# arkCyber/whisper-rust

Measured on AMD Instinct MI355X. Metric: real-time factor (audio-sec/wall-sec), greedy, 30 s synthetic chunks, higher is better.
Workload: dtype f16 operands / f32 accumulate; 1 GPU; ggml-small-shaped synthetic F16 model, greedy best_of=1 temperature_inc=0, 1 x 30 s 16 kHz f32 chunk per GPU, PCM resident in HBM; flash_attn=False, parallelism=chunk-dp1

## Files before the change

### whisper-rust_amd/csrc/wa_device.h

```cpp
#pragma once
#include "wa_kernels.h"

#include <hip/hip_runtime.h>
#include <stdint.h>

typedef _Float16 h16;
typedef _Float16 half8 __attribute__((ext_vector_type(8)));
typedef _Float16 half2v __attribute__((ext_vector_type(2)));
typedef float    f32x4 __attribute__((ext_vector_type(4)));

#define WAVE 64

__device__ __forceinline__ float h2f(wa_f16 v) { union { wa_f16 u; h16 h; } c; c.u = v; return (float) c.h; }
__device__ __forceinline__ wa_f16 f2h(float v) { asm("" : "+v"(v)); union { wa_f16 u; h16 h; } c; c.h = (h16) v; return c.u; }

__device__ __forceinline__ void wa_barrier_lds() { asm volatile("s_waitcnt lgkmcnt(0)\n\ts_barrier" ::: "memory"); }

__device__ __forceinline__ float wave_sum(float v) {
#pragma unroll
    for (int o = 32; o > 0; o >>= 1) v += __shfl_xor(v, o, WAVE);
    return v;
}
template <int CTRL, int ROW_MASK = 0xf>
__device__ __forceinline__ float dpp_f32(float v) {
// ... 3 lines not shown
__device__ __forceinline__ double dpp_f64(double v) {
    const long long b = __builtin_bit_cast(long long, v);
    const int lo = __builtin_amdgcn_update_dpp(0, (int) (b & 0xffffffffll), CTRL, ROW_MASK, 0xf, true);
    const int hi = __builtin_amdgcn_update_dpp(0, (int) (b >> 32), CTRL, ROW_MASK, 0xf, true);
    return __builtin_bit_cast(double, ((long long) hi << 32) | (unsigned int) lo);
}
__device__ __forceinline__ double wave_sum_d(double v) {
    v += dpp_f64<0x111>(v);
    v += dpp_f64<0x112>(v);
    v += dpp_f64<0x114>(v);
    v += dpp_f64<0x118>(v);
    v += dpp_f64<0x142, 0xa>(v);
    v += dpp_f64<0x143, 0xc>(v);
    const long long b = __builtin_bit_cast(long long, v);
    const int lo = __builtin_amdgcn_readlane((int) (b & 0xffffffffll), 63), hi = __builtin_amdgcn_readlane((int) (b >> 32), 63);
    return __builtin_bit_cast(double, ((long long) hi << 32) | (unsigned int) lo);
}
__device__ __forceinline__ float wave_max(float v) {
#pragma unroll
    for (int o = 32; o > 0; o >>= 1) v = fmaxf(v, __shfl_xor(v, o, WAVE));
    return v;
}

__device__ __forceinline__ float wa_expf(float x) {
    const float r = 0x1.8p23f;
    const float z = fmaf(x, 0x1.715476p+0f, r);
    const float n = z - r;
    const float b = fmaf(-n, 0x1.7f7d1cp-20f, fmaf(-n, 0x1.62e4p-1f, x));
    const uint32_t e = __float_as_uint(z) << 23;
    const float k = __uint_as_float(e + __float_as_uint(1.0f));
    const float an = fabsf(n);
    const float u = b * b;
    const float j = fmaf(fmaf(fmaf(0x1.0e4020p-7f, b, 0x1.573e2ep-5f), u, fmaf(0x1.555e66p-3f, b, 0x1.fffdb6p-2f)), u,
                         0x1.ffffecp-1f * b);
    if (!(an > 126.0f)) return fmaf(j, k, k);
    const uint32_t g = (n <= 0.0f) ? 0x82000000u : 0u;
    const float s1 = __uint_as_float(g + 0x7f000000u);
    const float s2 = __uint_as_float(e - g);
    if (an > 192.0f) return s1 * s1;
    return fmaf(s2, j, s2) * s1;
}

__device__ __forceinline__ float wa_gelu_nb(float x, const wa_f16 * __restrict__ table) {
    const float t = h2f(table[f2h(x)]);
    return x <= -10.0f ? 0.0f : (x >= 10.0f ? x : t);
}
__device__ __forceinline__ float wa_gelu(float x, const wa_f16 * __restrict__ table) {
    if (x <= -10.0f) return 0.0f;
    if (x >=  10.0f) return x;
    return h2f(table[f2h(x)]);
}

__device__ __forceinline__ void wa_q8_store(float y, int row, int blk, int el, int nb, int8_t * __restrict__ qs, float * __restrict__ qd,
                                            float * __restrict__ qsum = nullptr) {
    float a = fabsf(y);
    a = fmaxf(a, dpp_f32<0x128>(a));
    a = fmaxf(a, dpp_f32<0x124>(a));
    a = fmaxf(a, dpp_f32<0x122>(a));
    a = fmaxf(a, dpp_f32<0x121>(a));
    a = fmaxf(a, __shfl_xor(a, 16, 32));
    const float d = a / 127.f;
    const float id = a != 0.0f ? 127.f / a : 0.0f;
    const int q = (int) rintf(y * id);
    qs[(((size_t) row * 8 + (el >> 2)) * nb + blk) * 4 + (el & 3)] = (int8_t) q;
    if (el == 0) qd[(size_t) row * nb + blk] = h2f(f2h(d));
    if (qsum) {
        int t = q;
        t += __builtin_amdgcn_update_dpp(0, t, 0x128, 0xf, 0xf, true);
        t += __builtin_amdgcn_update_dpp(0, t, 0x124, 0xf, 0xf, true);
        t += __builtin_amdgcn_update_dpp(0, t, 0x122, 0xf, 0xf, true);
        t += __builtin_amdgcn_update_dpp(0, t, 0x121, 0xf, 0xf, true);
        t += __shfl_xor(t, 16, 32);
        if (el == 0) qsum[(size_t) row * nb + blk] = h2f(f2h(d * (float) t));
    }
}

struct wa_epi_pre { float bias = 0.f, scale = 1.f, resid = 0.f; };

template <int EPI>
__device__ __forceinline__ wa_epi_pre epi_preload(const wa_epi & e, int m, int n) {
    wa_epi_pre p;
    if (e.bias) p.bias = e.bias[n];
    if ((EPI == WA_EPI_F16 || EPI == WA_EPI_CROSS_KV || EPI == WA_EPI_DEC_QKV) && e.scale) p.scale = e.scale[n];
    if (EPI == WA_EPI_RESID || EPI == WA_EPI_CONV2) p.resid = e.resid[(size_t) m * e.ldr + n];
    return p;
}

template <int EPI>
__device__ __forceinline__ void epi_apply(const wa_epi & e, int m, int n, float acc, const wa_epi_pre & p) {
    float v = acc;
    if (e.bias) v = v + p.bias;
    if (EPI == WA_EPI_F16) {
        if (e.scale) v = v * p.scale;
        ((wa_f16 *) e.out)[(size_t) m * e.ldo + n] = f2h(v);
    } else if (EPI == WA_EPI_ENC_QKV) {
        if (n < e.split0) ((wa_f16 *) e.out)[(size_t) m * e.ldo + n] = f2h(v);
        else              ((wa_f16 *) e.out2)[(size_t) (n - e.split0) * e.ldo2 + m] = f2h(v);
    } else if (EPI == WA_EPI_GELU_F16) {
        ((wa_f16 *) e.out)[(size_t) m * e.ldo + n] = f2h(wa_gelu(v, e.gelu));
    } else if (EPI == WA_EPI_GELU_F32) {
        ((float *) e.out)[(size_t) m * e.ldo + n] = wa_gelu(v, e.gelu);
    } else if (EPI == WA_EPI_RESID) {
        ((float *) e.out)[(size_t) m * e.ldo + n] = v + p.resid;
    } else if (EPI == WA_EPI_CONV2) {
        const float g = wa_gelu(v, e.gelu);
        if (e.dbg) e.dbg[(size_t) m * e.ldo + n] = g;
        ((float *) e.out)[(size_t) m * e.ldo + n] = p.resid + g;
    } else if (EPI == WA_EPI_F32) {
        ((float *) e.out)[(size_t) m * e.ldo + n] = v;
    } else if (EPI == WA_EPI_CROSS_KV) {
        if (e.scale) v = v * p.scale;
        const int d = e.aux1, two_d = 2 * d;
        const int il = n / two_d, r = n - il * two_d;
        const int kv = r >= d, rr = kv ? r - d : r;
        const int n_head = d >> 6, hd = rr >> 6, c = rr & 63;
        wa_f16 * dst = (wa_f16 *) (kv ? e.out2 : e.out);
        dst[(((size_t) il * n_head + hd) * e.aux0 + m) * 64 + c] = f2h(v);
    } else if (EPI == WA_EPI_DEC_QKV) {
        if (e.scale) v = v * p.scale;
        const int row_off = e.dyn ? e.dyn[1] : e.row_off;
        if (n < e.split0)      ((wa_f16 *) e.out)[(size_t) m * e.ldo + n] = f2h(v);
        else if (e.rowp) {
            const wa_rowptr r = e.rowp[m];
            if (n < e.split1) (r.kv_k + e.rowp_off)[(size_t) r.kv_head * e.ldo2 + (n - e.split0)] = f2h(v);
            else              (r.kv_v + e.rowp_off)[(size_t) r.kv_head * e.ldo3 + (n - e.split1)] = f2h(v);
        }
        else if (n < e.split1) ((wa_f16 *) e.out2)[(size_t) (row_off + m) * e.ldo2 + (n - e.split0)] = f2h(v);
        else                   ((wa_f16 *) e.out3)[(size_t) (row_off + m) * e.ldo3 + (n - e.split1)] = f2h(v);
    }
}

template <int EPI>
__device__ __forceinline__ void epi_store(const wa_epi & e, int m, int n, float acc) {
    epi_apply<EPI>(e, m, n, acc, epi_preload<EPI>(e, m, n));
}

__device__ __forceinline__ float wa_tree32(const float (&s)[32]) {
    float a[8];
#pragma unroll
    for (int l = 0; l < 8; ++l) a[l] = (s[l] + s[16 + l]) + (s[8 + l] + s[24 + l]);
    const float t0 = a[0] + a[4], t1 = a[1] + a[5], t2 = a[2] + a[6], t3 = a[3] + a[7];
    return (t0 + t1) + (t2 + t3);
}

static __device__ const unsigned long long WA_EXP2F_T[32] = {
    0x3ff0000000000000ULL, 0x3fefd9b0d3158574ULL, 0x3fefb5586cf9890fULL, 0x3fef9301d0125b51ULL, 0x3fef72b83c7d517bULL,
    0x3fef54873168b9aaULL, 0x3fef387a6e756238ULL, 0x3fef1e9df51fdee1ULL, 0x3fef06fe0a31b715ULL, 0x3feef1a7373aa9cbULL,
    0x3feedea64c123422ULL, 0x3feece086061892dULL, 0x3feebfdad5362a27ULL, 0x3feeb42b569d4f82ULL, 0x3feeab07dd485429ULL,
    0x3feea47eb03a5585ULL, 0x3feea09e667f3bcdULL, 0x3fee9f75e8ec5f74ULL, 0x3feea11473eb0187ULL, 0x3feea589994cce13ULL,
    0x3feeace5422aa0dbULL, 0x3feeb737b0cdc5e5ULL, 0x3feec49182a3f090ULL, 0x3feed503b23e255dULL, 0x3feee89f995ad3adULL,
    0x3feeff76f2fb5e47ULL, 0x3fef199bdd85529cULL, 0x3fef3720dcef9069ULL, 0x3fef5818dcfba487ULL, 0x3fef7c97337b9b5fULL,
    0x3fefa4afa2a490daULL, 0x3fefd0765b6e4540ULL,
};
__device__ __forceinline__ float wa_expf_libm(float x) {
    if (!(x >= -0x1.9fe368p6f)) return 0.0f;
    const double InvLn2N = 0x1.71547652b82fep+0 * 32;
    const double C0 = 0x1.c6af84b912394p-5 / 32 / 32 / 32, C1 = 0x1.ebfce50fac4f3p-3 / 32 / 32, C2 = 0x1.62e42ff0c52d6p-1 / 32;
    const double SHIFT = 0x1.8p+52;
    double z = InvLn2N * (double) x;
    double kd = z + SHIFT;
    const unsigned long long ki = (unsigned long long) __double_as_longlong(kd);
    kd = kd - SHIFT;
    const double r = z - kd;
    const unsigned long long t = WA_EXP2F_T[ki & 31] + (ki << 47);
    const double s = __longlong_as_double((long long) t);
    z = fma(C0, r, C1);
    const double r2 = r * r;
    double y = fma(C2, r, 1.0);
    y = fma(z, r2, y);
    y = y * s;
    return (float) y;
}

__device__ __forceinline__ bool wa_sum_bounds(double S, double A, int n, float & lo, float & hi, double rn) {
    const double delta = (2.0 * (double) n * 0x1p-53 * A + fabs(S) * 0x1p-48) * rn * 1.000001;
    const double q = S * rn;
    lo = (float) (q - delta); hi = (float) (q + delta);
    return lo == hi;
}
__device__ __forceinline__ bool wa_sum_certain(double S, double A, int n, float & out, double rn) { float hi; return wa_sum_bounds(S, A, n, out, hi, rn); }
__device__ __forceinline__ bool wa_sum_certain(double S, double A, int n, float & out) { return wa_sum_certain(S, A, n, out, 1.0 / (double) n); }
__device__ __forceinline__ bool wa_mean_indifferent(float x, float lo, float hi) { return (x - lo) == (x - hi); }

__device__ __forceinline__ void wa_softmax_bounds(double tot, int ng, float & ilo, float & ihi) {
    const double delta = (double) (ng + 8 + 16) * 0x1p-53 * tot * 1.000001;
    ilo = (float) (1.0 / (tot + delta)); ihi = (float) (1.0 / (tot - delta));
}

__device__ __forceinline__ double wa_seq_sum_lds(const float * row, int d, bool squares, float mean) {
    double t = 0.0;
    int i = 0;
    for (; i + 4 <= d; i += 4) {
        const float4 v = *(const float4 *) (row + i);
        if (!squares) { t += (double) v.x; t += (double) v.y; t += (double) v.z; t += (double) v.w; }
        else {
            const float a = v.x - mean, b = v.y - mean, c = v.z - mean, e = v.w - mean;
            t += (double) (a * a); t += (double) (b * b); t += (double) (c * c); t += (double) (e * e);
        }
    }
    for (; i < d; ++i) { const float a = row[i] - mean; t += squares ? (double) (a * a) : (double) row[i]; }
    return t;
}
```

### whisper-rust_amd/csrc/wa_mega.hip

```cpp
#include "wa_one_launch_dev.h"
#include "wa_mega.h"

typedef const __attribute__((address_space(4))) wa_mega_args * mg_kargs;

#define MG_THREADS 512
#define MG_NW (MG_THREADS / 64)
#define MG_NP3 4

__device__ __forceinline__ int mq_fresh(int) {
    unsigned z = 0; asm volatile("" : "+v"(z));
    return (int) __builtin_amdgcn_mbcnt_hi(~0u, __builtin_amdgcn_mbcnt_lo(~0u, z));
}
__device__ __forceinline__ void mq_put(float y, bool act, unsigned * q32, float * dsc, int lane) {
    float dq;
    const unsigned w = mq_quant32(y, dq);
    if (act && (lane & 3) == 0) *q32 = w;
    if (act && (lane & 31) == 0) *dsc = dq;
}

__device__ __forceinline__ gu64 * mg_edge(mg_kargs A, int layer, int e) {
    return (gu64 *) A->granules + ((size_t) layer * WA_MEGA_EDGES + e) * A->edge_stride;
}

__device__ __forceinline__ int8_t * mq_xq(wa_f16 * xin) { return (int8_t *) xin; }
// ... 750 lines not shown
                    v = v + t.bias;
                    float gl = v;
                    if (v <= -10.0f) gl = 0.0f; else if (v < 10.0f) gl = h2f(gelu_l[t.valid ? f2h(v) : 0]);
                    if constexpr (Q) { if (t.valid && (lane & 7) == 0) gr_store(eh + t.row, seq, __float_as_uint(gl)); }
                    else mg_pub_h2(eh, seq, t.valid, t.row, (unsigned) f2h(gl), lane);
                }
                mg_trace(A, wg == 0 && wave == 1 && lane == 0, (l * 8 + 4) * 8 + 3, mg_now());
                if ((wave == 3 || wave == 4) && wave - 1 < g_ff) big_next(wave);
                else if (wave >= 6 && l + 1 >= L) mg_prefetch_logits<NS, Q>(A, pf, have_pf, lane, wave);
            }
        } else
        if (wave == 1 || wave == 2 || (BIG && (wave == 3 || wave == 4))) {
            bool assisted = false;
            gu64 * eh = mg_edge(A, l, E_HF);
            for (int grp = wave - 1; grp < g_ff; grp += BIG ? 4 : 2) {
                if (grp >= 2) { t = mg_mk8<Q, NS>(pf, Y.fc1_w, Y.fc1_d, Y.fc1_b, nullptr, d4, d, row_ff, r_ff, grp, lane); assisted = true; }
                MG_CHAOS_AT(7u);
                float v = mg_do8<Q, NS>(pf, t, d >> 5, xinB, lane);
                v = v + t.bias;
                float gl = v;
                if (v <= -10.0f) gl = 0.0f; else if (v < 10.0f) gl = h2f(gelu_l[t.valid ? f2h(v) : 0]);
                if constexpr (Q) { if (t.valid && (lane & 7) == 0) gr_store(eh + t.row, seq, __float_as_uint(gl)); }
                else mg_pub_h2(eh, seq, t.valid, t.row, (unsigned) f2h(gl), lane);
            }
            mg_trace(A, wg == 0 && wave == 1 && lane == 0, (l * 8 + 4) * 8 + 3, mg_now());
            if (A->dbg && l == MG_WGTRACE_LAYER) mg_trace(A, wave == 1 && lane == 0, 4096 + wg * 8 + 6, mg_now());
            if (CQ) {
                if (l + 1 >= L) mg_prefetch_logits<NS, Q>(A, pf, have_pf, lane, wave);
            } else if (assisted) {
                if (l + 1 >= L) mg_prefetch_logits<NS, Q>(A, pf, have_pf, lane, wave);
                else t = wave == 3 ? mg_mk8<Q, NS>(pf, Ly[l + 1].out_w, Ly[l + 1].out_d, Ly[l + 1].out_b, nullptr, d, d, row_d, r_d, 0, lane)
                                   : mg_mk8<Q, NS>(pf, Ly[l + 1].cq_w, Ly[l + 1].cq_d, Ly[l + 1].cq_b, nullptr, d, d, row_d, r_d, 0, lane);
            }
        }
        MG_FRESH();
        {
            const int ng = QB ? 9 * (d4 >> 5) : Q ? d4 : 2 * d;
            const int qs = mg_slot(wave, QB || BIG ? MG_EX_HFQ : MG_EX_HF), sg = mg_seg(ng), i0 = qs * sg, i1 = min(ng, i0 + sg);
            if constexpr (QB) { if (qs >= 0) mg_gather_qb<3>(c, mg_edge(A, l, E_HF), i0, i1, lane, xin, d4 >> 5, 600u + l, A, wg == 0 && wave == 0 ? (l * 8 + 5) * 8 : -1); }
            else if constexpr (Q) { if (qs >= 0) mg_gather_q8<(NP3 == MG_NP3 ? 14 : 8)>(c, mg_edge(A, l, E_HF), i0, i1, lane, xin, d4 >> 5, 600u + l, A, wg == 0 && wave == 0 ? (l * 8 + 5) * 8 : -1); }
            else if (qs >= 0) mg_gather_h2<7>(c, mg_edge(A, l, E_HF), i0, i1, lane, (unsigned *) xin, 600u + l, A, wg == 0 && wave == 0 ? (l * 8 + 5) * 8 : -1);
        }
        wa_barrier_lds();
        MG_FRESH();
        mg_trace(A, wg == 0 && wave == 5 && lane == 0, (l * 8 + 5) * 8 + 4, mg_now());
        if (!CQ && (wave == 1 || wave == 2)) {
            if (l + 1 < L) t = mg_mk8<Q, NS>(pf, Ly[l + 1].qkv_w, Ly[l + 1].qkv_d, Ly[l + 1].qkv_b, Ly[l + 1].qkv_s, 3 * d, d, row_qkv, r_qkv, wave - 1, lane);
            else mg_prefetch_logits<NS, Q>(A, pf, have_pf, lane, wave);
        }
        if (wave == 5 || (BIG && (wave == 3 || wave == 4))) {
            const bool own = !BIG || wave == 5;
            bool assisted = false;
            gu64 * ex = mg_edge(A, l, E_X3);
            for (int grp = own ? 0 : wave - 2; grp < g_d16; grp += BIG ? 3 : 1) {
                if (grp >= (BIG ? 3 : 1)) t = mg_mk16<Q, 4 * NS>(pf, Y.fc2_w, Y.fc2_d, Y.fc2_b, d, d4, row_d, r_d, grp, lane);
                if (grp >= 1) assisted = true;
                MG_CHAOS_AT(8u);
                float v = mg_do16<Q, 4 * NS>(pf, t, d4 >> 5, xin, lane);
                v = v + t.bias;
                if (t.valid && (lane & 15) == MG_RES16(Q)) gr_store(ex + t.row, seq, __float_as_uint(v + xf[t.row]));
            }
            mg_trace(A, wg == 0 && own && lane == 0, (l * 8 + 5) * 8 + 3, mg_now());
            if (own && l + 1 >= L) mg_prefetch_logits<NS, Q>(A, pf, have_pf, lane, wave);
            else if (assisted) {
                if (l + 1 >= L) mg_prefetch_logits<NS, Q>(A, pf, have_pf, lane, wave);
                else t = wave == 3 ? mg_mk8<Q, NS>(pf, Ly[l + 1].out_w, Ly[l + 1].out_d, Ly[l + 1].out_b, nullptr, d, d, row_d, r_d, 0, lane)
                                   : mg_mk8<Q, NS>(pf, Ly[l + 1].cq_w, Ly[l + 1].cq_d, Ly[l + 1].cq_b, nullptr, d, d, row_d, r_d, 0, lane);
            }
        }
    }
    if (L == 0 && wave >= 1 && wave <= 5) mg_prefetch_logits<NS, Q>(A, pf, have_pf, lane, wave);
    MG_FRESH();
    mg_final<NP3, NS, Q>(A, c, smem, pf, have_pf, gw, gb, lane, wave);
#undef MG_FRESH
}

struct mg_att_smem { float * sc; wa_f16 * p16; float * gs; float * red; double * redd; float * s_inv; wa_f16 * qs; float * part; };
__device__ __forceinline__ mg_att_smem mg_att_carve(unsigned char * base, int maxkv) {
    mg_att_smem m;
    m.redd = (double *) base;                       base += 8 * sizeof(double);
    m.sc   = (float *) base;                        base += (size_t) maxkv * 4;
    m.gs   = (float *) base;                        base += (size_t) (maxkv / 8) * 4;
    m.part = (float *) base;                        base += 32 * 64 * 4;
    m.red  = (float *) base;                        base += 8 * 4;
    m.s_inv = (float *) base;                       base += 4 * 4;
    m.p16  = (wa_f16 *) base;                       base += (size_t) maxkv * 2;
    m.qs   = (wa_f16 *) base;
    return m;
}


template <bool Q = false>
__device__ __forceinline__ void mg_attn_finish(const float * part, const wa_f16 * vleft , const wa_f16 * p16, int np, int nl,
                                               gu64 * edge, int h, unsigned seq, int tid, double * dbl0, double * dbl1 ,
                                               mg_kargs A = nullptr, int tslot = -1) {
    asm volatile("" : "+s"(nl));
    if (tid >= 64) {
        const int wv = tid >> 6, o = tid & 63;
        float nzero = -0.0f;
        asm volatile("" : "+v"(nzero));
#pragma unroll
        for (int i = 0; i < 5; ++i) {
            const int cc = 5 * (wv - 1) + i;
            if (cc < 32) {
                const float pr = fmaf(h2f(vleft[cc * 64 + o]), h2f((p16 + np)[cc]), nzero);
                (cc < 16 ? dbl0 : dbl1)[(cc & 15) * 64 + o] = (double) (cc < nl ? pr : -0.0f);
            }
        }
    }
    double sumf = 0.0;
    if (tid < 64) {
        if (tslot >= 0) mg_trace(A, tid == 0, tslot, mg_now());
        float s32[32];
#pragma unroll
        for (int r = 0; r < 32; ++r) s32[r] = part[r * 64 + tid];
        sumf = (double) wa_tree32(s32);
        if (tslot >= 0) mg_trace(A, tid == 0, tslot + 1, mg_now() + (sumf == 1e300 ? 1u : 0u));
    }
    wa_barrier_lds();
    if (tid < 64) {
        double dv[32];
#pragma unroll
        for (int cc = 0; cc < 32; ++cc) dv[cc] = (cc < 16 ? dbl0 : dbl1)[(cc & 15) * 64 + tid];
        __builtin_amdgcn_sched_barrier(0);
#pragma unroll
        for (int cc = 0; cc < 32; ++cc) sumf += dv[cc];
        if (tslot >= 0) mg_trace(A, tid == 0, tslot + 2, mg_now() + (sumf == 1e300 ? 1u : 0u));
        mo_attn_publish<Q>((float) sumf, edge, h, seq, tid);
    }
}

__device__ __forceinline__ void mg_attn_finish16(const float * part, const double * dbl, gu64 * edge, int o0, unsigned seq, int tid,
                                                 mg_kargs A = nullptr, int tslot = -1) {
    if (tid < 16) {
        if (tslot >= 0) mg_trace(A, tid == 0, tslot, mg_now());
        float s32[32];
        double dv[32];
#pragma unroll
        for (int r = 0; r < 32; ++r) s32[r] = part[r * 16 + tid];
#pragma unroll
        for (int cc = 0; cc < 32; ++cc) dv[cc] = dbl[cc * 16 + tid];
        __builtin_amdgcn_sched_barrier(0);
        double sumf = (double) wa_tree32(s32);
        if (tslot >= 0) mg_trace(A, tid == 0, tslot + 1, mg_now() + (sumf == 1e300 ? 1u : 0u));
#pragma unroll
        for (int cc = 0; cc < 32; ++cc) sumf += dv[cc];
        if (tslot >= 0) mg_trace(A, tid == 0, tslot + 2, mg_now() + (sumf == 1e300 ? 1u : 0u));
        const unsigned hv = (unsigned) f2h((float) sumf);
        const unsigned hi = dpp_u32<0x101>(hv);
        if ((tid & 1) == 0) gr_store(edge + ((o0 + tid) >> 1), seq, (hv & 0xffffu) | (hi << 16));
    }
}

template <bool Q = false>
__device__ __forceinline__ void mg_role_self(mg_kargs A_, int idx_) {
    extern __shared__ __attribute__((aligned(16))) unsigned char smem[];
    const mg_kargs A = mo_uniform(A_);
    const int tid = threadIdx.x, lane = tid & 63;
    const int wave = __builtin_amdgcn_readfirstlane(tid >> 6);
    const int h = __builtin_amdgcn_readfirstlane(idx_);
    mo_ctl c; c.status = (gu32 *) A->status; c.seq = A->seq; c.dead = false;
    mg_chaos_start(c.seq);

    wa_f16 * Ks = (wa_f16 *) smem;
    wa_f16 * Vs = Ks + WA_MEGA_MAX_KV * 64;
    const mg_att_smem M = mg_att_carve(smem + (size_t) WA_MEGA_MAX_KV * 64 * 2 * 2, WA_MEGA_MAX_KV);
    const int d = A->d, n_kv = A->n_kv, kv_head = A->kv_head, L = A->n_layer;
    const int a = tid & 3, kslot = tid >> 2;
    if (wave == 0) mg_pick(A, lane, (int *) (smem + MG_PICK_OFF));
    for (int l = 0; l < L; ++l) {
        {
            const gch kc = (gch) A->kv_k + (size_t) l * A->kv_layer_stride + h * 64;
            const gch vc = (gch) A->kv_v + (size_t) l * A->kv_layer_stride + h * 64;
            const int n16 = n_kv * 8;
            u32x4 tk[8], tv[8];
#pragma unroll
            for (int j = 0; j < 8; ++j) {
                const int idx = tid + MG_THREADS * j;
                if (idx < n16) {
                    tk[j] = *(const GAS u32x4 *) (kc + (size_t) (idx >> 3) * d + (idx & 7) * 8);
                    tv[j] = *(const GAS u32x4 *) (vc + (size_t) (idx >> 3) * d + (idx & 7) * 8);
                }
            }
#pragma unroll
            for (int j = 0; j < 8; ++j) {
                const int idx = tid + MG_THREADS * j;
                if (idx < n16) { *(u32x4 *) (Ks + (size_t) idx * 8) = tk[j]; *(u32x4 *) (Vs + (size_t) idx * 8) = tv[j]; }
            }
        }
        wa_barrier_lds();
        if (wave == 0) {
            unsigned v[2];
            const unsigned sp = mo_sweep<MO_POLL_OWN, 2>(mg_edge(A, l, E_QKV), [&](int k) {
                if (k == 0) return (lane < 32 ? 0 : (d >> 1)) + h * 32 + (lane & 31);
                return lane < 32 ? d + h * 32 + lane : -1; }, c, lane, v, 1000u + l);
            mg_trace(A, h == 0 && lane == 0, (l * 8 + 6) * 8 + 0, mg_now()); mg_trace(A, h == 0 && lane == 0, (l * 8 + 6) * 8 + 1, sp);
            if (lane < 32) { ((unsigned *) M.qs)[lane] = v[0]; ((unsigned *) (Vs + (size_t) kv_head * 64))[lane] = v[1]; }
            else ((unsigned *) (Ks + (size_t) kv_head * 64))[lane - 32] = v[0];
        }
        wa_barrier_lds();
        float lmax = -INFINITY;
        {
            float qa[8], qb[8];
#pragma unroll
            for (int i = 0; i < 8; ++i) { qa[i] = h2f(M.qs[8 * a + i]); qb[i] = h2f(M.qs[32 + 8 * a + i]); }
            for (int c0 = 0; c0 < n_kv; c0 += MG_THREADS / 4) {
                const int cc = c0 + kslot, cl = cc < n_kv ? cc : n_kv - 1;
                const u32x4 ka = *(const u32x4 *) (Ks + (size_t) cl * 64 + 8 * a), kb = *(const u32x4 *) (Ks + (size_t) cl * 64 + 32 + 8 * a);
                const float r = mo_score(ka, kb, qa, qb, 1.0f);
                if (cc < n_kv) { if (a == 0) M.sc[cc] = r; lmax = fmaxf(lmax, r); }
            }
        }
        mg_trace(A, h == 0 && tid == 0, (l * 8 + 6) * 8 + 4, mg_now());
        {
            lmax = wave_max(lmax);
            if (lane == 0) M.red[wave] = lmax;
            wa_barrier_lds();
            float mx = M.red[0];
#pragma unroll
            for (int k = 1; k < MG_NW; ++k) mx = fmaxf(mx, M.red[k]);
            const int n8 = n_kv & ~7, ng = n8 >> 3;
            float e = 0.0f;
            double ps = 0.0;
            if (tid < n_kv) e = tid < n8 ? wa_expf(M.sc[tid] - mx) : wa_expf_libm(M.sc[tid] - mx);
            {
                float t = e + dpp_f32<0x104>(e);
                t = t + dpp_f32<0x102>(t);
                t = t + dpp_f32<0x101>(t);
                if (tid < n8) ps = (tid & 7) == 0 ? (double) t : 0.0;
                else if (tid < n_kv) ps = (double) e;
            }
            ps = wave_sum_d(ps);
            if (lane == 0) M.redd[wave] = ps;
            wa_barrier_lds();
            const double tot = ((M.redd[0] + M.redd[1]) + (M.redd[2] + M.redd[3])) + ((M.redd[4] + M.redd[5]) + (M.redd[6] + M.redd[7]));
            float ilo, ihi;
            wa_softmax_bounds(tot, ng, ilo, ihi);
            if (ilo != ihi && tid == 0 && !c.dead) __hip_atomic_store(c.status, (unsigned) WA_MEGA_REDO, __ATOMIC_RELAXED, __HIP_MEMORY_SCOPE_AGENT);
            if (tid < n_kv) M.p16[tid] = f2h(e * ilo);
            wa_barrier_lds();
        }
        mg_trace(A, h == 0 && tid == 0, (l * 8 + 6) * 8 + 5, mg_now());
        MG_CHAOS_ID(1000 + h, 21u, c.seq);
        const int np = n_kv & ~31, nsteps = np >> 5;
        {
            float acc[4] = { 0.0f, 0.0f, 0.0f, 0.0f };
            const int r0 = wave * 4;
            for (int s = 0; s < nsteps; ++s) {
#pragma unroll
                for (int i = 0; i < 4; ++i)
                    acc[i] = fmaf(h2f(Vs[(size_t) (s * 32 + r0 + i) * 64 + lane]), h2f(M.p16[s * 32 + r0 + i]), acc[i]);
            }
#pragma unroll
            for (int i = 0; i < 4; ++i) M.part[(r0 + i) * 64 + lane] = acc[i];
        }
        wa_barrier_lds();
        mg_attn_finish<Q>(M.part, Vs + (size_t) np * 64, M.p16, np, n_kv - np, mg_edge(A, l, E_AO), h, c.seq, tid, (double *) (Ks + WA_MEGA_KV_ROOM * 64),
                          (double *) (Vs + WA_MEGA_KV_ROOM * 64), A, A->dbg && h == 0 && l == MG_WGTRACE_LAYER ? 3004 : -1);
        mg_trace(A, h == 0 && tid == 0, (l * 8 + 6) * 8 + 3, mg_now());
        wa_barrier_lds();
    }
    unsigned pf[96];
    bool have_pf = false;
    float gw[MG_NP3], gb[MG_NP3];
    if (wave >= 1) mg_prefetch_logits<0, Q>(A, pf, have_pf, lane, wave);
    mg_ln_params<MG_NP3>(gw, gb, A->lnf_w, A->lnf_b, A->d, mg_slot(wave, MG_EX_FINAL), lane);
    mg_final<MG_NP3, 0, Q>(A, c, smem, pf, have_pf, gw, gb, lane, wave);
}

#define MG_CSTEPS 48
#define MG_CGR 2048
#define MG_CGR_MAX 0
#define MG_CGR_SUM 8
#define MG_CGR_XCC 16
#define MG_CGR_PART 64
#define MG_CGR_XCC1 WA_MEGA_MAX_T
#define MG_CP_LD 56
#define MG_CX_XF 32768
#define MG_CX_XIN (MG_CX_XF + WA_MEGA_MAX_D * 4)
#define MG_CX_LNRED (MG_CX_XIN + WA_MEGA_MAX_D * 2)
#define MG_CX_END (MG_CX_LNRED + 256)
#define MG_CX_TRACE 6144

template <bool Q = false, int CQ = -1, bool X1 = false>
__device__ __forceinline__ void mg_role_cross(mg_kargs A_, int idx_) {
    static_assert(!X1 || (CQ >= 0 && !Q), "the one-exchange form is the F16 d = 768 kernel's");
    extern __shared__ __attribute__((aligned(16))) unsigned char smem[];
    const mg_kargs A = mo_uniform(A_);
    int tid = threadIdx.x, lane = tid & 63;
    const int wave = __builtin_amdgcn_readfirstlane(tid >> 6);
    const int H = A->n_head;
    const int ci = __builtin_amdgcn_readfirstlane(idx_);
    const int h = ci >> 2, w = ci & 3;
    mo_ctl c; c.status = (gu32 *) A->status; c.seq = A->seq; c.dead = false;
    mg_chaos_start(c.seq);
    const unsigned seq = c.seq;

    float  * part  = (float *) smem;
    wa_f16 * vleft = (wa_f16 *) (smem + 8192);
    float  * sc    = (float *) (smem + 8192 + 4096);
    wa_f16 * p16   = (wa_f16 *) (smem + 8192 + 4096 + 1536);
    wa_f16 * pleft = (wa_f16 *) (smem + 8192 + 4096 + 1536 + 768);
    wa_f16 * qs    = (wa_f16 *) (smem + 8192 + 4096 + 1536 + 768 + 64);
    double * redd  = (double *) (smem + 8192 + 4096 + 1536 + 768 + 64 + 128);
    float  * red   = (float *) (smem + 8192 + 4096 + 1536 + 768 + 64 + 128 + 64);
    float  * bc    = red + 8;
    double * dbl   = nullptr;
    if constexpr (X1) {
        constexpr int o_sc = 0, o_p16 = o_sc + WA_MEGA_MAX_T * 4, o_part = o_p16 + 32 * MG_CP_LD * 2, o_dbl = o_part + 32 * 16 * 4, o_vleft = o_dbl + 32 * 16 * 8,
                      o_pleft = o_vleft + 32 * 16 * 2, o_qs = o_pleft + 32 * 2, o_redd = o_qs + 64 * 2, o_red = o_redd + 8 * 8, o_bc = o_red + 8 * 4, o_end = o_bc + 4 * 4;
        static_assert(o_end <= MG_CX_XF && o_p16 % 16 == 0 && o_dbl % 8 == 0 && o_vleft % 16 == 0 && o_redd % 8 == 0 && MG_CP_LD % 8 == 0 && MG_CP_LD >= MG_CSTEPS,
                      "LDS of the one-exchange form: below the role's LayerNorm area, 16-byte rows where 16 bytes are read");
        sc    = (float *) (smem + o_sc);
        p16   = (wa_f16 *) (smem + o_p16);
        part  = (float *) (smem + o_part);
        dbl   = (double *) (smem + o_dbl);
        vleft = (wa_f16 *) (smem + o_vleft);
        pleft = (wa_f16 *) (smem + o_pleft);
        qs    = (wa_f16 *) (smem + o_qs);
        redd  = (double *) (smem + o_redd);
        red   = (float *) (smem + o_red);
        bc    = (float *) (smem + o_bc);
    }

    const int T = A->T, tpad = A->cross_tpad, L = A->n_layer;
    const float kq_scale = A->kq_scale;
    int a = tid & 3, ks = tid >> 2;
    const int np = T & ~31, nsteps = np >> 5, nl = T - np, n8 = T & ~7, ng = n8 >> 3;
    if (wave == 0) mg_pick(A, lane, (int *) (smem + MG_PICK_OFF));
    if (wave == 0) {
        const unsigned xcc = (unsigned) __builtin_amdgcn_s_getreg(20 | (3 << 11)) & 0xfu;
        gu64 * X0 = (gu64 *) A->cross_gr + (size_t) h * MG_CGR + (X1 ? MG_CGR_XCC1 : MG_CGR_XCC);
        if (lane == 0) gr_store(X0 + w, seq, xcc);
        unsigned v[1];
        mo_sweep<MO_POLL_OWN, 1>(X0, [&](int) { return lane < 4 ? lane : -1; }, c, lane, v, 2900u);
        const bool same = lane >= 4 || v[0] == xcc;
        if (lane == 0) bc[2] = __builtin_amdgcn_ballot_w64(same) == ~0ull && !c.dead ? 1.0f : 0.0f;
    }
    wa_barrier_lds();
    const bool local = bc[2] != 0.0f;
    const __attribute__((address_space(4))) wa_mega_layer * Ly = (const __attribute__((address_space(4))) wa_mega_layer *) A->layers;
    float  * xf    = (float *) (smem + MG_CX_XF);
    wa_f16 * xin   = (wa_f16 *) (smem + MG_CX_XIN);
    double * lnred = (double *) (smem + MG_CX_LNRED);
    const int d = A->d;
    for (int l = 0; l < L; ++l) {
        if constexpr (CQ >= 0) {
            unsigned z = threadIdx.x; asm volatile("" : "+v"(z));
            tid = (int) z; lane = tid & 63; a = tid & 3; ks = tid >> 2;
        }
        gu64 * X = (gu64 *) A->cross_gr + ((size_t) l * H + h) * MG_CGR;
        const gch kp = (gch) A->cross_k + (size_t) l * A->cross_layer_stride + (size_t) h * tpad * 64;
        const gch vp = (gch) A->cross_v + (size_t) l * A->cross_layer_stride + (size_t) h * tpad * 64;
        u32x4 ka[3], kb[3];
        unsigned short vv[MG_CSTEPS];
#pragma unroll
        for (int p = 0; p < 3; ++p) {
            const int o = p * 128 + ks, cc = 32 * (o >> 3) + 8 * w + (o & 7);
            if (cc < T) { ka[p] = *(const GAS u32x4 *) (kp + (size_t) cc * 64 + 8 * a); kb[p] = *(const GAS u32x4 *) (kp + (size_t) cc * 64 + 32 + 8 * a); }
        }
        if constexpr (X1) {
#pragma unroll
            for (int s = 0; s < MG_CSTEPS; ++s) if (s < nsteps) vv[s] = *(const GAS unsigned short *) (vp + (size_t) (32 * s + (tid >> 4)) * 64 + 16 * w + (tid & 15));
            if (wave == 0) {
                const int row = tid >> 1;
                if (row < nl) *(u32x4 *) (vleft + (size_t) tid * 8) = *(const GAS u32x4 *) (vp + (size_t) (np + row) * 64 + 16 * w + (tid & 1) * 8);
            }
        } else {
#pragma unroll
        for (int s = 0; s < MG_CSTEPS; ++s) if (s < nsteps) vv[s] = *(const GAS unsigned short *) (vp + (size_t) (32 * s + 8 * w + wave) * 64 + lane);
        if (w == 0 && tid < 256) {
            const int row = tid >> 3;
            if (row < nl) *(u32x4 *) (vleft + (size_t) tid * 8) = *(const GAS u32x4 *) (vp + (size_t) (np + row) * 64 + (tid & 7) * 8);
        }
        }
        if constexpr (CQ >= 0) {
            unsigned pf[96];
            float gw[2], gb[2];
            const int row = 64 * h + 8 * wave + (lane >> 3);
            const gch wrow = (gch) Ly[l].cq_w + (size_t) row * d + 4 * (lane & 7);
            mg_pf8<CQ>(pf, wrow, true, d >> 5, 0);
            const float bias = ((gcf) Ly[l].cq_b)[row];
            mg_ln_params<2>(gw, gb, Ly[l].ln2_w, Ly[l].ln2_b, d, mg_slot(wave, 0u), lane);
            mg_trace(A, ci == 0 && lane == 0 && wave == 0, (l * 8 + 7) * 8 + 2, mg_now());
            mg_ln3<2>(A, c, mg_edge(A, l, E_X1), gw, gb, mg_slot(wave, 0u), lane, xf, xin, lnred, 2000u + l,
                      ci == 0 && wave == 0 ? MG_CX_TRACE + l * 8 : -1);
            MG_CHAOS_ID(2000 + ci, 30u, seq);
            float v = mg_dot8<CQ>(pf, wrow, true, d >> 5, xin, lane & 7, true);
            v = v + bias;
            const unsigned hq = (unsigned) f2h(v);
            if ((lane & 7) == 0) qs[8 * wave + (lane >> 3)] = (wa_f16) hq;
            if (A->dbg && w == 0) mg_pub_h2(mg_edge(A, l, E_QC), seq, true, row, hq, lane);
            mg_trace(A, ci == 0 && lane == 0 && wave == 0, (l * 8 + 7) * 8 + 0, mg_now());
            if (A->dbg && l == MG_WGTRACE_LAYER && w == 0) mg_trace(A, tid == 0, 3200 + h, mg_now());
        } else if (wave == 0) {
            unsigned v[1];
            mg_trace(A, ci == 0 && lane == 0, (l * 8 + 7) * 8 + 2, mg_now());
            const unsigned sp = mo_sweep<MO_POLL_OWN, 1>(mg_edge(A, l, E_QC), [&](int) { return lane < 32 ? h * 32 + lane : -1; }, c, lane, v, 2000u + l);
            mg_trace(A, ci == 0 && lane == 0, (l * 8 + 7) * 8 + 0, mg_now()); mg_trace(A, ci == 0 && lane == 0, (l * 8 + 7) * 8 + 1, sp);
            if (A->dbg && l == MG_WGTRACE_LAYER && w == 0) mg_trace(A, lane == 0, 3200 + h, mg_now());
            if (lane < 32) ((unsigned *) qs)[lane] = v[0];
        }
        wa_barrier_lds();
#define MG_CX(k) do { if (A->dbg && l == MG_WGTRACE_LAYER) mg_trace(A, ci == 0 && tid == 0, 3010 + (k), mg_now()); } while (0)
        if constexpr (X1) {
        MG_CX(0);
        MG_CHAOS_ID(2000 + ci, 31u, seq);
        float lmax = -INFINITY;
        {
// ... 122 lines not shown
            float g = lane < 4 ? __uint_as_float(v[0]) : -INFINITY;
            g = fmaxf(g, dpp_f32<0x4e>(g)); g = fmaxf(g, dpp_f32<0xb1>(g));
            if (lane == 0) bc[0] = g;
            MG_CX(3);
        }
        wa_barrier_lds();
        mg_trace(A, ci == 0 && tid == 0, (l * 8 + 7) * 8 + 4, mg_now());
        const float mx = bc[0];
        {
            double ps = 0.0;
            if (tid < 8 * MG_CSTEPS) {
                const int g = 4 * (tid >> 3) + w, cc = 8 * g + (tid & 7);
                const float e = cc < n8 ? wa_expf(sc[tid] - mx) : (cc < T ? wa_expf_libm(sc[tid] - mx) : 0.0f);
                sc[tid] = e;
                float t = e + dpp_f32<0x104>(e);
                t = t + dpp_f32<0x102>(t);
                t = t + dpp_f32<0x101>(t);
                if (g < ng) ps = (tid & 7) == 0 ? (double) t : 0.0;
                else ps = (double) e;
            }
            ps = wave_sum_d(ps);
            if (lane == 0) redd[wave] = ps;
        }
        MG_CX(4);
        wa_barrier_lds();
        if (wave == 0) {
            const double ps = ((redd[0] + redd[1]) + (redd[2] + redd[3])) + ((redd[4] + redd[5]) + (redd[6] + redd[7]));
            const u64 pb = (u64) __double_as_longlong(ps);
            if (lane == 0) { gr_store_l(X + MG_CGR_SUM + 2 * w, seq, (unsigned) pb, local); gr_store_l(X + MG_CGR_SUM + 2 * w + 1, seq, (unsigned) (pb >> 32), local); }
            unsigned v[1];
            mo_sweep<MO_POLL_OWN, 1>(X + MG_CGR_SUM, [&](int) { return lane < 8 ? lane : -1; }, c, lane, v, 2200u + l);
            double tot = 0.0;
#pragma unroll
            for (int k = 0; k < 4; ++k) {
                const unsigned lo = __builtin_amdgcn_readlane(v[0], 2 * k), hi = __builtin_amdgcn_readlane(v[0], 2 * k + 1);
                tot += __longlong_as_double((long long) (((u64) hi << 32) | lo));
            }
            float ilo, ihi;
            wa_softmax_bounds(tot, ng, ilo, ihi);
            if (ilo != ihi && lane == 0 && !c.dead) __hip_atomic_store(c.status, (unsigned) WA_MEGA_REDO, __ATOMIC_RELAXED, __HIP_MEMORY_SCOPE_AGENT);
            if (lane == 0) bc[1] = ilo;
            MG_CX(5);
        }
        wa_barrier_lds();
        mg_trace(A, ci == 0 && tid == 0, (l * 8 + 7) * 8 + 5, mg_now());
        const float inv = bc[1];
        if (tid < 8 * MG_CSTEPS) {
            const int cc = 32 * (tid >> 3) + 8 * w + (tid & 7);
            if (cc < T) {
                const wa_f16 ph = f2h(sc[tid] * inv);
                p16[(tid & 7) * MG_CSTEPS + (tid >> 3)] = ph;
                if (cc >= np) { if (w == 0) pleft[cc - np] = ph; else gr_store_l(X + MG_CGR_PART + (w - 1) * 576 + 512 + (tid & 7), seq, (unsigned) ph, local); }
            }
        }
        wa_barrier_lds();
        MG_CX(6);
        MG_CHAOS_ID(2000 + ci, 32u, seq);
        {
            float acc = 0.0f;
            half8 pw[MG_CSTEPS / 8];
#pragma unroll
            for (int k = 0; k < MG_CSTEPS / 8; ++k) pw[k] = *(const half8 *) (p16 + wave * MG_CSTEPS + 8 * k);
#pragma unroll
            for (int s = 0; s < MG_CSTEPS; ++s) if (s < nsteps) acc = fmaf(h2f(vv[s]), (float) pw[s >> 3][s & 7], acc);
            if (w == 0) part[wave * 64 + lane] = acc;
            else gr_store_l(X + MG_CGR_PART + (w - 1) * 576 + wave * 64 + lane, seq, __float_as_uint(acc), local);
        }
        mg_trace(A, ci == 0 && tid == 0, (l * 8 + 7) * 8 + 6, mg_now());
        if (w == 0) {
            if (wave >= 1 && wave <= 6) {
                const int ww = (wave - 1) >> 1, half = (wave - 1) & 1;
                gu64 * src = X + MG_CGR_PART + ww * 576;
                unsigned v[5];
                mo_sweep<MO_POLL_OWN, 5>(src, [&](int k) { return k < 4 ? half * 256 + 64 * k + lane : (half == 0 && lane < 8 && 8 * (ww + 1) + lane < nl ? 512 + lane : -1); }, c, lane, v, 2300u + l);
#pragma unroll
                for (int k = 0; k < 4; ++k) part[(8 * (ww + 1) + 4 * half + k) * 64 + lane] = __uint_as_float(v[k]);
                if (half == 0 && lane < 8) { const int cc = 8 * (ww + 1) + lane; if (cc < nl) pleft[cc] = (wa_f16) v[4]; }
            }
            wa_barrier_lds();
            mg_trace(A, ci == 0 && tid == 0, (l * 8 + 7) * 8 + 7, mg_now());
            mg_attn_finish<Q>(part, vleft, pleft - np, np, nl, mg_edge(A, l, E_AO2), h, seq, tid, (double *) (smem + 16384), (double *) (smem + 24576), A,
                              A->dbg && ci == 0 && l == MG_WGTRACE_LAYER ? 3000 : -1);
            mg_trace(A, ci == 0 && tid == 0, (l * 8 + 7) * 8 + 3, mg_now());
            if (A->dbg && l == MG_WGTRACE_LAYER) mg_trace(A, tid == 0, 3100 + h, mg_now());
        }
        }
        wa_barrier_lds();
    }
    unsigned pf[96];
    bool have_pf = false;
    float gw[MG_NP3], gb[MG_NP3];
    if (wave >= 1) mg_prefetch_logits<0, Q>(A, pf, have_pf, lane, wave);
    mg_ln_params<MG_NP3>(gw, gb, A->lnf_w, A->lnf_b, A->d, mg_slot(wave, MG_EX_FINAL), lane);
    mg_final<MG_NP3, 0, Q>(A, c, smem, pf, have_pf, gw, gb, lane, wave);
}

#ifndef MG_CQ_TU
__global__ __launch_bounds__(MG_THREADS) void k_decode_mega(const wa_mega_args A) {
    int role, idx;
    mg_role_of((int) gridDim.x, A.n_head, (int) blockIdx.x, role, idx);
    const mg_kargs Ap = (mg_kargs) __builtin_amdgcn_kernarg_segment_ptr();
    if (role == 0) {
        if (A.d == 768) mg_role_gemv<2, 24>(Ap, idx); else if (A.d < 768) mg_role_gemv<2, 0>(Ap, idx);
        else mg_role_gemv<MG_NP3, 0>(Ap, idx);
    }
    else if (role == 1) mg_role_self(Ap, idx);
    else                mg_role_cross(Ap, idx);
}


__global__ __launch_bounds__(MG_THREADS) void k_decode_mega_q(const wa_mega_args A) {
    int role, idx;
    mg_role_of((int) gridDim.x, A.n_head, (int) blockIdx.x, role, idx);
    const mg_kargs Ap = (mg_kargs) __builtin_amdgcn_kernarg_segment_ptr();
    if (role == 0) {
        if (A.d == 768) mg_role_gemv<2, 24, true>(Ap, idx); else if (A.d < 768) mg_role_gemv<2, 0, true>(Ap, idx);
        else if (A.d == 1280) mg_role_gemv<MG_NP3, 40, true>(Ap, idx); else mg_role_gemv<MG_NP3, 0, true>(Ap, idx);
    }
    else if (role == 1) mg_role_self<true>(Ap, idx);
    else                mg_role_cross<true>(Ap, idx);
}

size_t wa_mega_lds_bytes() {
    const size_t s_self  = (size_t) WA_MEGA_MAX_KV * 64 * 2 * 2 + MG_ATT_SMEM(WA_MEGA_MAX_KV);
    const size_t s_cross = MG_CX_END;
    const size_t s_gemv  = MG_PICK_OFF;
    size_t m = s_self > s_cross ? s_self : s_cross;
    m = m > s_gemv ? m : s_gemv;
    if (m > MG_PICK_OFF || (MG_PICK_OFF & 255) != 0) abort();
    return MG_PICK_OFF + MG_PICK_BYTES;
}

bool wa_launch_decode_mega(hipStream_t s, const wa_mega_args & a, int n_wg) {
    static bool attr_set[64] = {};
    const size_t lds = wa_mega_lds_bytes();
    int dev = 0;
    (void) hipGetDevice(&dev);
    if (!attr_set[dev & 63]) {
        if (hipFuncSetAttribute((const void *) k_decode_mega, hipFuncAttributeMaxDynamicSharedMemorySize, (int) lds) != hipSuccess ||
            hipFuncSetAttribute((const void *) k_decode_mega_q, hipFuncAttributeMaxDynamicSharedMemorySize, (int) lds) != hipSuccess) return false;
        attr_set[dev & 63] = true;
    }
    if (!a.quant && a.d == 768) return wa_launch_decode_mega_cq(s, a, n_wg, lds);
    if (a.quant) hipLaunchKernelGGL(k_decode_mega_q, dim3(n_wg), dim3(MG_THREADS), lds, s, a);
    else         hipLaunchKernelGGL(k_decode_mega, dim3(n_wg), dim3(MG_THREADS), lds, s, a);
    return hipGetLastError() == hipSuccess;
}
#else
__global__ __launch_bounds__(MG_THREADS) void k_decode_mega_cq(const wa_mega_args A) {
    int role, idx;
    mg_role_of((int) gridDim.x, A.n_head, (int) blockIdx.x, role, idx);
    const mg_kargs Ap = (mg_kargs) __builtin_amdgcn_kernarg_segment_ptr();
    if (role == 0)      mg_role_gemv<2, 24, false, true>(Ap, idx);
    else if (role == 1) mg_role_self(Ap, idx);
    else                mg_role_cross<false, 24, true>(Ap, idx);
}

bool wa_launch_decode_mega_cq(hipStream_t s, const wa_mega_args & a, int n_wg, size_t lds) {
    static bool attr_set[64] = {};
    int dev = 0;
    (void) hipGetDevice(&dev);
    if (!attr_set[dev & 63]) {
        if (hipFuncSetAttribute((const void *) k_decode_mega_cq, hipFuncAttributeMaxDynamicSharedMemorySize, (int) lds) != hipSuccess) return false;
        attr_set[dev & 63] = true;
    }
    hipLaunchKernelGGL(k_decode_mega_cq, dim3(n_wg), dim3(MG_THREADS), lds, s, a);
    return hipGetLastError() == hipSuccess;
}
#endif
```

Before: 360.8 x real-time.

## Add fast self-attention path with single-wave scoring and packed P·V loop

Adds an NF template path to the self-attention role in the d=768 decode megakernel. When n_kv ≤ 64, scoring runs in one wave with a bpermute transpose and max/sum reductions inside the wave, which removes several workgroup barriers. The P·V accumulation is rewritten to load packed half2 V and P values in unrolled blocks of four. The exp lookup table is copied into LDS for the tail elements. This adds code complexity and relies on exact rounding matching the old path so the bounds checks stay valid.

```diff
diff --git a/whisper-rust_amd/csrc/wa_device.h b/whisper-rust_amd/csrc/wa_device.h
--- a/whisper-rust_amd/csrc/wa_device.h
+++ b/whisper-rust_amd/csrc/wa_device.h
@@ -179,7 +179,7 @@
     0x3feeff76f2fb5e47ULL, 0x3fef199bdd85529cULL, 0x3fef3720dcef9069ULL, 0x3fef5818dcfba487ULL, 0x3fef7c97337b9b5fULL,
     0x3fefa4afa2a490daULL, 0x3fefd0765b6e4540ULL,
 };
-__device__ __forceinline__ float wa_expf_libm(float x) {
+__device__ __forceinline__ float wa_expf_libm_tab(float x, const unsigned long long * tab) {
     if (!(x >= -0x1.9fe368p6f)) return 0.0f;
     const double InvLn2N = 0x1.71547652b82fep+0 * 32;
     const double C0 = 0x1.c6af84b912394p-5 / 32 / 32 / 32, C1 = 0x1.ebfce50fac4f3p-3 / 32 / 32, C2 = 0x1.62e42ff0c52d6p-1 / 32;
@@ -189,7 +189,7 @@
     const unsigned long long ki = (unsigned long long) __double_as_longlong(kd);
     kd = kd - SHIFT;
     const double r = z - kd;
-    const unsigned long long t = WA_EXP2F_T[ki & 31] + (ki << 47);
+    const unsigned long long t = tab[ki & 31] + (ki << 47);
     const double s = __longlong_as_double((long long) t);
     z = fma(C0, r, C1);
     const double r2 = r * r;
@@ -198,6 +198,7 @@
     y = y * s;
     return (float) y;
 }
+__device__ __forceinline__ float wa_expf_libm(float x) { return wa_expf_libm_tab(x, WA_EXP2F_T); }
 
 __device__ __forceinline__ bool wa_sum_bounds(double S, double A, int n, float & lo, float & hi, double rn) {
     const double delta = (2.0 * (double) n * 0x1p-53 * A + fabs(S) * 0x1p-48) * rn * 1.000001;
diff --git a/whisper-rust_amd/csrc/wa_mega.hip b/whisper-rust_amd/csrc/wa_mega.hip
--- a/whisper-rust_amd/csrc/wa_mega.hip
+++ b/whisper-rust_amd/csrc/wa_mega.hip
@@ -926,7 +926,7 @@
     }
 }
 
-template <bool Q = false>
+template <bool Q = false, bool NF = false>
 __device__ __forceinline__ void mg_role_self(mg_kargs A_, int idx_) {
     extern __shared__ __attribute__((aligned(16))) unsigned char smem[];
     const mg_kargs A = mo_uniform(A_);
@@ -942,6 +942,7 @@
     const int d = A->d, n_kv = A->n_kv, kv_head = A->kv_head, L = A->n_layer;
     const int a = tid & 3, kslot = tid >> 2;
     if (wave == 0) mg_pick(A, lane, (int *) (smem + MG_PICK_OFF));
+    if constexpr (NF) { if (tid < 32) ((unsigned long long *) M.gs)[tid] = WA_EXP2F_T[tid]; }
     for (int l = 0; l < L; ++l) {
         {
             const gch kc = (gch) A->kv_k + (size_t) l * A->kv_layer_stride + h * 64;
@@ -972,6 +973,86 @@
             if (lane < 32) { ((unsigned *) M.qs)[lane] = v[0]; ((unsigned *) (Vs + (size_t) kv_head * 64))[lane] = v[1]; }
             else ((unsigned *) (Ks + (size_t) kv_head * 64))[lane - 32] = v[0];
         }
+        if constexpr (NF) {
+        const bool one = n_kv <= 64;
+        if (!one) wa_barrier_lds();
+        else asm volatile("" ::: "memory");
+        MG_CHAOS_ID(1000 + h, 22u, c.seq);
+        const bool has = 64 * wave < n_kv;
+        float r = -INFINITY, lmax = -INFINITY;
+        if (!one || wave == 0) {
+            float qa[8], qb[8];
+#pragma unroll
+            for (int i = 0; i < 8; ++i) { qa[i] = h2f(M.qs[8 * a + i]); qb[i] = h2f(M.qs[32 + 8 * a + i]); }
+            if (one) {
+                float rj[4] = { 0.0f, 0.0f, 0.0f, 0.0f };
+#pragma unroll
+                for (int j = 0; j < 4; ++j) {
+                    if (16 * j < n_kv) {
+                        const int cc = 16 * j + (lane >> 2), cl = cc < n_kv ? cc : n_kv - 1;
+                        const u32x4 ka = *(const u32x4 *) (Ks + (size_t) cl * 64 + 8 * a), kb = *(const u32x4 *) (Ks + (size_t) cl * 64 + 32 + 8 * a);
+                        rj[j] = mo_score(ka, kb, qa, qb, 1.0f);
+                    }
+                }
+                const float mine = a == 0 ? rj[0] : a == 1 ? rj[1] : a == 2 ? rj[2] : rj[3];
+                const float got = __builtin_bit_cast(float, __builtin_amdgcn_ds_bpermute(4 * (4 * (lane & 15) + (lane >> 4)), __builtin_bit_cast(int, mine)));
+                if (tid < n_kv) r = lmax = got;
+            } else {
+                for (int c0 = 0; c0 < n_kv; c0 += MG_THREADS / 4) {
+                    const int cc = c0 + kslot, cl = cc < n_kv ? cc : n_kv - 1;
+                    const u32x4 ka = *(const u32x4 *) (Ks + (size_t) cl * 64 + 8 * a), kb = *(const u32x4 *) (Ks + (size_t) cl * 64 + 32 + 8 * a);
+                    const float sc = mo_score(ka, kb, qa, qb, 1.0f);
+                    if (cc < n_kv) { if (a == 0) M.sc[cc] = sc; lmax = fmaxf(lmax, sc); }
+                }
+            }
+        }
+        mg_trace(A, h == 0 && tid == 0, (l * 8 + 6) * 8 + 4, mg_now());
+        MG_CHAOS_ID(1000 + h, 23u, c.seq);
+        {
+            lmax = fmaxf(lmax, dpp_f32<0x128>(lmax)); lmax = fmaxf(lmax, dpp_f32<0x124>(lmax));
+            lmax = fmaxf(lmax, dpp_f32<0x122>(lmax)); lmax = fmaxf(lmax, dpp_f32<0x121>(lmax));
+            {
+                const int b = __builtin_bit_cast(int, lmax);
+                const float m0 = __builtin_bit_cast(float, __builtin_amdgcn_readlane(b, 0)), m1 = __builtin_bit_cast(float, __builtin_amdgcn_readlane(b, 16));
+                const float m2 = __builtin_bit_cast(float, __builtin_amdgcn_readlane(b, 32)), m3 = __builtin_bit_cast(float, __builtin_amdgcn_readlane(b, 48));
+                lmax = fmaxf(fmaxf(m0, m1), fmaxf(m2, m3));
+            }
+            float mx = lmax;
+            if (!one) {
+                if (lane == 0) M.red[wave] = lmax;
+                wa_barrier_lds();
+                mx = M.red[0];
+#pragma unroll
+                for (int k = 1; k < MG_NW; ++k) mx = fmaxf(mx, M.red[k]);
+                if (tid < n_kv) r = M.sc[tid];
+            }
+            const int n8 = n_kv & ~7, ng = n8 >> 3;
+            float e = 0.0f;
+            double ps = 0.0;
+            if (has) {
+                if (tid < n_kv) e = tid < n8 ? wa_expf(r - mx) : wa_expf_libm_tab(r - mx, (const unsigned long long *) M.gs);
+                float t = e + dpp_f32<0x104>(e);
+                t = t + dpp_f32<0x102>(t);
+                t = t + dpp_f32<0x101>(t);
+                if (tid < n8) ps = (tid & 7) == 0 ? (double) t : 0.0;
+                else if (tid < n_kv) ps = (double) e;
+                ps = wave_sum_d(ps);
+            }
+            double tot = ps;
+            if (!one) {
+                if (lane == 0) M.redd[wave] = ps;
+                wa_barrier_lds();
+                tot = ((M.redd[0] + M.redd[1]) + (M.redd[2] + M.redd[3])) + ((M.redd[4] + M.redd[5]) + (M.redd[6] + M.redd[7]));
+            }
+            if (has) {
+                float ilo, ihi;
+                wa_softmax_bounds(tot, ng, ilo, ihi);
+                if (ilo != ihi && tid == 0 && !c.dead) __hip_atomic_store(c.status, (unsigned) WA_MEGA_REDO, __ATOMIC_RELAXED, __HIP_MEMORY_SCOPE_AGENT);
+                if (tid < n_kv) M.p16[tid] = f2h(e * ilo);
+            }
+            wa_barrier_lds();
+        }
+        } else {
         wa_barrier_lds();
         float lmax = -INFINITY;
         {
@@ -1014,9 +1095,44 @@
             if (tid < n_kv) M.p16[tid] = f2h(e * ilo);
             wa_barrier_lds();
         }
+        }
         mg_trace(A, h == 0 && tid == 0, (l * 8 + 6) * 8 + 5, mg_now());
         MG_CHAOS_ID(1000 + h, 21u, c.seq);
         const int np = n_kv & ~31, nsteps = np >> 5;
+        if constexpr (NF) {
+        {
+            const int r0 = wave * 4, hw = lane >> 5, o2 = lane & 31;
+            float acc[2][2] = { { 0.0f, 0.0f }, { 0.0f, 0.0f } };
+            const wa_f16 * vbase = Vs + (size_t) (r0 + hw) * 64 + 2 * o2;
+            auto block = [&](auto nk, int s0) {
+                constexpr int NK = decltype(nk)::value;
+                unsigned va[NK], vb[NK];
+                u32x2 pp[NK];
+#pragma unroll
+                for (int k = 0; k < NK; ++k) {
+                    va[k] = *(const unsigned *) (vbase + (size_t) (s0 + k) * 32 * 64);
+                    vb[k] = *(const unsigned *) (vbase + (size_t) (s0 + k) * 32 * 64 + 2 * 64);
+                    pp[k] = *(const u32x2 *) (M.p16 + (s0 + k) * 32 + r0);
+                }
+                __builtin_amdgcn_sched_barrier(0);
+#pragma unroll
+                for (int k = 0; k < NK; ++k) {
+                    const float pa = h2f((wa_f16) (hw ? pp[k].x >> 16 : pp[k].x & 0xffffu)), pb = h2f((wa_f16) (hw ? pp[k].y >> 16 : pp[k].y & 0xffffu));
+                    acc[0][0] = fmaf(h2f((wa_f16) (va[k] & 0xffffu)), pa, acc[0][0]); acc[0][1] = fmaf(h2f((wa_f16) (va[k] >> 16)), pa, acc[0][1]);
+                    acc[1][0] = fmaf(h2f((wa_f16) (vb[k] & 0xffffu)), pb, acc[1][0]); acc[1][1] = fmaf(h2f((wa_f16) (vb[k] >> 16)), pb, acc[1][1]);
+                }
+            };
+            int s0 = 0;
+            for (; s0 + 4 <= nsteps; s0 += 4) block(std::integral_constant<int, 4>(), s0);
+            const int rem = nsteps - s0;
+            if (rem == 3) block(std::integral_constant<int, 3>(), s0);
+            else if (rem == 2) block(std::integral_constant<int, 2>(), s0);
+            else if (rem == 1) block(std::integral_constant<int, 1>(), s0);
+            *(float2 *) (M.part + (r0 + hw) * 64 + 2 * o2) = make_float2(acc[0][0], acc[0][1]);
+            *(float2 *) (M.part + (r0 + 2 + hw) * 64 + 2 * o2) = make_float2(acc[1][0], acc[1][1]);
+        }
+        mg_trace(A, h == 0 && tid == 0, (l * 8 + 6) * 8 + 6, mg_now());
+        } else {
         {
             float acc[4] = { 0.0f, 0.0f, 0.0f, 0.0f };
             const int r0 = wave * 4;
@@ -1028,7 +1144,9 @@
 #pragma unroll
             for (int i = 0; i < 4; ++i) M.part[(r0 + i) * 64 + lane] = acc[i];
         }
-        wa_barrier_lds();
+        }
+        wa_barrier_lds();
+        if constexpr (NF) mg_trace(A, h == 0 && tid == 0, (l * 8 + 6) * 8 + 7, mg_now());
         mg_attn_finish<Q>(M.part, Vs + (size_t) np * 64, M.p16, np, n_kv - np, mg_edge(A, l, E_AO), h, c.seq, tid, (double *) (Ks + WA_MEGA_KV_ROOM * 64),
                           (double *) (Vs + WA_MEGA_KV_ROOM * 64), A, A->dbg && h == 0 && l == MG_WGTRACE_LAYER ? 3004 : -1);
         mg_trace(A, h == 0 && tid == 0, (l * 8 + 6) * 8 + 3, mg_now());
@@ -1457,7 +1575,7 @@
     mg_role_of((int) gridDim.x, A.n_head, (int) blockIdx.x, role, idx);
     const mg_kargs Ap = (mg_kargs) __builtin_amdgcn_kernarg_segment_ptr();
     if (role == 0)      mg_role_gemv<2, 24, false, true>(Ap, idx);
-    else if (role == 1) mg_role_self(Ap, idx);
+    else if (role == 1) mg_role_self<false, true>(Ap, idx);
     else                mg_role_cross<false, 24, true>(Ap, idx);
 }
 
```

New measurement: 367.0 x real-time, median of 6. 1.7% higher.
